# matinmoezzi/MyCobotGym

Hardware: AMD Instinct MI355X
Metric: env-steps/sec (whole node), MyCobot Reach, N_envs=8192/GPU (higher is better)
Workload: dtype f64

## Files before the change

### mycobotgym_amd/csrc/mcg_dynamics.hpp

```cpp
#pragma once
#ifndef MCG_DUP
#define MCG_DUP 0
#endif

#include <type_traits>
#include <hip/hip_runtime.h>
#include "mcg.h"

namespace mcg {

typedef double real;

constexpr int NB = 12;
constexpr int AXK[NB] = {2, 0, 0, 0, 2, 0, 1, 1, 1, 1, 1, 1};
constexpr int AXS[NB] = {-1, -1, 1, -1, -1, -1, 1, -1, -1, 1, 1, 1};
constexpr int PAR[NB] = {-1, 0, 1, 2, 3, 4, 5, 6, 5, 8, 5, 5};
constexpr real MINVAL = 1e-15, MINIMP = 1e-4, MAXIMP = 0.9999;

#define MCG_DEV __device__ __forceinline__

enum { ST_LOAD = 0, ST_CTRL, ST_TRIG, ST_RNE, ST_ACT, ST_CRB, ST_ROWS, ST_G0, ST_NEWTON, ST_EULER, ST_COLLIDE, ST_CUBE,
       ST_COUPLED, ST_CUBE_FIN, ST_POST, ST_N_BUILD, ST_N_FACTOR, ST_N_SOLVE, ST_N_CHECK, ST_E_RHS, ST_R_AX5, ST_R_CONNECT, ST_R_LIMITS, ST_C_MASK, ST_C_ASSEMBLE, ST_C_SCHUR, ST_C_SOLVE, ST_C_CHECK, ST_C_LS, ST_W2_WAIT1, ST_W2_COLLIDE, ST_W2_CUBE, ST_W2_WAIT2, ST_W1_WAIT, ST_A_ENTRY, ST_A_G, ST_A_TWIST, ST_A_LOOP, ST_A_MAP, ST_A_STORE,
       ST_CO_SETUP, ST_CO_ROWS, ST_CO_H0, ST_CO_RESID, ST_CO_ASM, ST_CO_FACTOR, ST_CO_SOLVE, ST_CO_CHECK, ST_CO_LS, ST_CO_OUT, ST_CO_IDLE,
       ST_X_S1C, ST_X_NUMBERS, ST_X_S2, ST_S_S1B, ST_S_MESH, ST_S_S1C, ST_S_NUMBERS,
// ... 117 lines not shown
  pc = fma(z, pc, T.t[11]); pc = fma(z, pc, T.t[12]);
  pc = fma(z, pc, T.t[13]); pc = fma(z, pc, T.t[14]);
  const real cr = fma(z * z, pc, fma(z, -0.5, 1.0));
  const int q = (int)k;
  const real s0 = (q & 1) ? cr : sr, c0 = (q & 1) ? sr : cr;
  s = (q & 2) ? -s0 : s0;
  c = ((q + 1) & 2) ? -c0 : c0;
}

MCG_DEV real impedance(const real* par, real dist) {
  const real d0 = par[2], dmax = par[3], width = par[4], mid = par[5], power = par[6];
  real imp;
  if (d0 == dmax || width <= MINVAL) imp = 0.5 * (d0 + dmax);
  else {
    const real x = fabs(dist) * par[7];
    real y;
    if (power == 2) {
      const real u = 1 - x;
      y = (x <= mid) ? par[8] * (x * x) : 1 - par[9] * (u * u);
    } else y = x;
    imp = d0 + y * (dmax - d0);
    imp = (x >= 1) ? dmax : imp;
    imp = (x == 0) ? d0 : imp;
  }
  return fmin(fmax(imp, MINIMP), MAXIMP);
}

constexpr int tri(int i, int j) { return i >= j ? i * (i + 1) / 2 + j : j * (j + 1) / 2 + i; }

struct Pattern { bool nz[NB][NB]; };

constexpr bool is_ancestor_or_self(int a, int i) {
  while (i >= 0) { if (i == a) return true; i = PAR[i]; }
  return false;
}
constexpr Pattern symbolic(bool with_constraints, bool fill = true) {
  Pattern P{};
  for (int i = 0; i < NB; i++) for (int j = 0; j <= i; j++) P.nz[i][j] = is_ancestor_or_self(j, i);
  if (with_constraints) {
    constexpr int grp[2][3] = {{6, 7, 10}, {8, 9, 11}};
    for (int g = 0; g < 2; g++) for (int a = 0; a < 3; a++) for (int b = 0; b < 3; b++) {
      int i = grp[g][a], j = grp[g][b];
      if (i >= j) P.nz[i][j] = true;
    }
    for (int g = 0; g < 2; g++) for (int a = 0; a < 3; a++) for (int j = 0; j < 6; j++) P.nz[grp[g][a]][j] = true;
    P.nz[8][6] = true;
// ... 355 lines not shown
          for (int k = 0; k < 3; k++) cmc[p][k] += h3[k] + m * r[k];
          for (int k = 0; k < 6; k++) cI[p][k] += add[k];
        }
        pin(cm[p]); pin3(cmc[p]); pin6(cI[p]);
      }
      asm volatile("" ::: "memory");
      MCG_FENCE();
    });
}

template <class LS>
MCG_DEV void euler_accel(ModelPtr Pm, real h, const LS MS, const real* a, real* rhs) {
  real Mh[NB * (NB + 1) / 2], dinv[NB];
  static_for<NB>([&](auto I) { constexpr int i = I;
    static_for<i + 1>([&](auto Jj) { constexpr int j = Jj; if constexpr (PAT_M.nz[i][j]) Mh[tri(i, j)] = MS.ld(LDS_M + tri(i, j)); }); });
  static_for<NB>([&](auto I) { constexpr int i = I; real sacc = 0;
    static_for<NB>([&](auto Jj) { constexpr int j = Jj;
      if constexpr (PAT_M.nz[i > j ? i : j][i > j ? j : i]) sacc = fma(Mh[tri(i, j)], a[j], sacc); }); rhs[i] = sacc; });
  { ModelPtr Q = launder(Pm); static_for<NB>([&](auto I) { constexpr int i = I; Mh[tri(i, i)] = fma(h, Q->body[i].damping, Mh[tri(i, i)]); }); }
  ldl_factor<PAT_M>(Mh, dinv);
  ldl_solve<PAT_M>(Mh, dinv, rhs);
}

struct NoSplit { static constexpr bool enabled = false, rne_remote = false, factor_remote = false, early_heq = false, warm_lds = false, mesh_split = false, solve_remote = false,
                                       trig_once = false;
                 static constexpr int QB = 0, QDB = 0, FS = 0, WARM = 0, QLAG = 0; };
struct SplitMain { static constexpr bool enabled = true, rne_remote = true, factor_remote = true, early_heq = true, warm_lds = true, mesh_split = false, solve_remote = true,
                                         trig_once = true;
                   static constexpr int QB = LDS_QB, QDB = LDS_QDB, FS = LDS_FS, WARM = LDS_WARM, QLAG = LDS_QLAG; };
struct SplitMainLocal : SplitMain { static constexpr bool solve_remote = false; };
struct SplitMainOwnTrig : SplitMain { static constexpr bool trig_once = false; };

template <int FIRST, class LS, class QF>
MCG_DEV void trig_exchange(const LS MS, QF q_of, real* sn, real* cs) {
  {
    const TrigC T = load_trig();
    static_for<4>([&](auto I) { constexpr int i = FIRST + I; real s, c; sincos_cw(T, AXS[i] * q_of(std::integral_constant<int, i>{}), s, c); MS.st(LDS_SN + i, s); MS.st(LDS_CS + i, c); });
  }
  __syncthreads();
  static_for<NB>([&](auto I) { constexpr int i = I; sn[i] = MS.ld(LDS_SN + i); cs[i] = MS.ld(LDS_CS + i); });
}

template <class SPL, class LS>
MCG_DEV void build_H(const LS MS, real* H, const bool* act_, const real* Dl) {
  static_for<NB>([&](auto I) { constexpr int i = I;
    static_for<i + 1>([&](auto Jj) { constexpr int j = Jj;
      if constexpr (PAT_E.nz[i][j]) {
        H[tri(i, j)] = MS.ld(LDS_HEQ + tri(i, j));
        if constexpr (SPL::early_heq && PAT_M.nz[i][j]) H[tri(i, j)] += MS.ld(LDS_M + tri(i, j));
      } else if constexpr (PAT_H.nz[i][j]) H[tri(i, j)] = 0.0; }); });
  static_for<10>([&](auto I) { constexpr int j = I; H[tri(j, j)] += act_[j] ? Dl[j] : 0.0; });
}

template <class SPL, class LS>
MCG_DEV bool no_other_rows(ModelPtr Pm, const LS MS) {
  real jr[10][2];
  { ModelPtr Q = launder(Pm); static_for<10>([&](auto I) { constexpr int j = I; if constexpr (j != 6 && j != 8) { jr[j][0] = Q->jnt_range[j][0]; jr[j][1] = Q->jnt_range[j][1]; } }); }
  bool other = false;
  static_for<10>([&](auto I) { constexpr int j = I;
// ... 22 lines not shown
  f0 = s0 * nu0; f1 = s1 * nu1;
}

MCG_DEV void gear_rows_solve(real* x, const real* z6, const real* z8, real Dl6, real arefl6, real sgl6, real Dl8, real arefl8, real sgl8) {
  const bool v6 = sgl6 != 0, v8 = sgl8 != 0, both = v6 && v8;
  const real D0 = v6 ? Dl6 : (v8 ? Dl8 : 1.0), D1 = both ? Dl8 : 1.0;
  const real ar0 = v6 ? arefl6 : arefl8, ar1 = both ? arefl8 : 0.0;
  const real s0 = v6 ? sgl6 : sgl8, s1 = both ? sgl8 : 0.0;
  const real xa0 = v6 ? x[6] : (v8 ? x[8] : 0.0), xa1 = both ? x[8] : 0.0;
  real W00 = v6 ? z6[6] : (v8 ? z8[8] : 0.0), W01 = both ? z6[8] : 0.0;
  const real W11 = both ? z8[8] : 0.0;
  W01 *= s0 * s1;
  const real rb0 = s0 * xa0 - ar0, rb1 = s1 * xa1 - ar1;
  real f0, f1;
  limit_pair(v6 || v8, both, D0, D1, s0, s1, rb0, rb1, W00, W01, W11, f0, f1);
  const real g6 = v6 ? f0 : 0.0, g8 = v6 ? f1 : f0;
  static_for<NB>([&](auto I) { constexpr int i = I; x[i] = fma(-z8[i], g8, fma(-z6[i], g6, x[i])); });
}

MCG_DEV bool bad_value(real x) { return !(fabs(x) <= 1e10); }

template <class LS, class CPL = NoCoupling, class WLD = NoWeld, class SPL = NoSplit, bool COMMIT = true>
MCG_DEV bool robot_substep(ModelPtr Pm, Robot& S, real* qlag6, const LS MS, CPL* CP = nullptr, const WLD* WD = nullptr,
                           Robot* next = nullptr) {
  MCG_COUNT(CN_SUBSTEP);
  if constexpr (SPL::enabled) __syncthreads();
  const real h = launder(Pm)->timestep;
  real cs[NB], sn[NB];
  if constexpr (SPL::trig_once) trig_exchange<0>(MS, [&](auto I) { return S.q[I]; }, sn, cs);
  else {
    const TrigC T = load_trig();
    static_for<NB>([&](auto I) { constexpr int i = I; sincos_cw(T, AXS[i] * S.q[i], sn[i], cs[i]); });
  }
  if constexpr (!(SPL::warm_lds && !CPL::enabled)) static_for<6>([&](auto I) { constexpr int i = I; qlag6[i] = S.q[i]; });
  static_for<NB>([&](auto I) { constexpr int i = I; pin(sn[i]); pin(cs[i]); });
  MCG_FENCE();

  MCG_TICK(ST_TRIG);
  real fs[NB];
  if constexpr (SPL::rne_remote) { static_for<NB>([&](auto I) { constexpr int i = I; fs[i] = 0; }); }
  else rne_bias(Pm, cs, sn, S.qd, fs);
  MCG_TICK(ST_RNE);
  {
    ModelPtr Q = launder(Pm);
    static_for<6>([&](auto I) {
      constexpr int u = I;
      real c = fmin(fmax(S.ctrl[u], Q->act_ctrlrange[u][0]), Q->act_ctrlrange[u][1]);
      real f = Q->act_gain[u] * c + Q->act_bias[u][0] + Q->act_bias[u][1] * S.q[u] + Q->act_bias[u][2] * S.qd[u];
      fs[u] += fmin(fmax(f, Q->act_forcerange[u][0]), Q->act_forcerange[u][1]);
    });
    const real c0 = Q->tendon_coef[0], c1 = Q->tendon_coef[1];
    real len = c0 * S.q[6] + c1 * S.q[8], vel = c0 * S.qd[6] + c1 * S.qd[8];
    real c = fmin(fmax(S.ctrl[6], Q->act_ctrlrange[6][0]), Q->act_ctrlrange[6][1]);
    real f = Q->act_gain[6] * c + Q->act_bias[6][0] + Q->act_bias[6][1] * len + Q->act_bias[6][2] * vel;
    f = fmin(fmax(f, Q->act_forcerange[6][0]), Q->act_forcerange[6][1]);
    fs[6] += c0 * f; fs[8] += c1 * f;
  }
  static_for<NB>([&](auto I) { constexpr int i = I; pin(fs[i]); });
  if constexpr (SPL::solve_remote) static_for<8>([&](auto K) { constexpr int k = K; MS.st(LDS_RACT + k, fs[RACT_DOF[k]]); });
  MCG_FENCE();

  MCG_TICK(ST_ACT);
  if constexpr (!SPL::enabled) crb_to_lds(Pm, cs, sn, MS);
  MCG_TICK(ST_CRB);
  real ax5[6][3];
  static_for<6>([&](auto I) {
    constexpr int i = I;
    for (int k = 0; k < 3; k++) ax5[i][k] = 0;
    ax5[i][AXK[i]] = AXS[i];
    static_for<5 - i>([&](auto Jj) {
      constexpr int j = i + 1 + Jj;
      real t[3]; rot_down<AXK[j]>(cs[j], sn[j], ax5[i], t);
      for (int k = 0; k < 3; k++) ax5[i][k] = t[k];
    });
  });
  MCG_TICK_PIN(ax5[0], 3); MCG_TICK_PIN(ax5[1], 3); MCG_TICK_PIN(ax5[2], 3); MCG_TICK_PIN(ax5[3], 3); MCG_TICK_PIN(ax5[4], 3);
  MCG_TICK(ST_R_AX5);
  real Jc[2][3][9];
  real Dc[2], arefc[2][3];
  static_for<2>([&](auto Sd) {
    constexpr int sd = Sd; constexpr int g = 6 + 2 * sd, fi = 7 + 2 * sd, hg = 10 + sd;
    ModelPtr Q = launder(Pm);
    real rg[3], rh[3], rf[3], an1[3], an2[3], par[10];
    ldc<3>(Q->body[g].r, rg); ldc<3>(Q->body[hg].r, rh); ldc<3>(Q->body[fi].r, rf);
    ldc<3>(Q->eq_anchor1[sd], an1); ldc<3>(Q->eq_anchor2[sd], an2); ldc<10>(Q->eq_par[sd], par);
    real t[3], t2[3], o_f[3], p1[3], p2[3];
    rot_up<1>(cs[g], sn[g], rf, t);
    for (int k = 0; k < 3; k++) o_f[k] = rg[k] + t[k];
    rot_up<1>(cs[fi], sn[fi], an1, t2); rot_up<1>(cs[g], sn[g], t2, t);
    for (int k = 0; k < 3; k++) p1[k] = o_f[k] + t[k];
    rot_up<1>(cs[hg], sn[hg], an2, t);
    for (int k = 0; k < 3; k++) p2[k] = rh[k] + t[k];
    const real pos[3] = {p1[0] - p2[0], p1[1] - p2[1], p1[2] - p2[2]};
    static_for<6>([&](auto I) { constexpr int i = I; real c3[3]; cross(ax5[i], pos, c3); for (int k = 0; k < 3; k++) Jc[sd][k][i] = c3[k]; });
    Jc[sd][0][6] = AXS[g] * (p1[2] - rg[2]);   Jc[sd][2][6] = -AXS[g] * (p1[0] - rg[0]);
    Jc[sd][0][7] = AXS[fi] * (p1[2] - o_f[2]); Jc[sd][2][7] = -AXS[fi] * (p1[0] - o_f[0]);
    Jc[sd][0][8] = -AXS[hg] * (p2[2] - rh[2]); Jc[sd][2][8] = AXS[hg] * (p2[0] - rh[0]);
    Jc[sd][1][6] = Jc[sd][1][7] = Jc[sd][1][8] = 0;
    const real imp = impedance(par, sqrt(dot3(pos, pos)));
    Dc[sd] = imp * rcp_nr(fmax(MINVAL * imp, (1 - imp) * Q->eq_diag[sd]));
    static_for<3>([&](auto Kk) {
      constexpr int k = Kk;
      real vel = 0;
      static_for<6>([&](auto I) { constexpr int i = I; vel = fma(Jc[sd][k][i], S.qd[i], vel); });
      if constexpr (k != 1) vel += Jc[sd][k][6] * S.qd[g] + Jc[sd][k][7] * S.qd[fi] + Jc[sd][k][8] * S.qd[hg];
      arefc[sd][k] = -par[1] * vel - par[0] * imp * pos[k];
    });
    pin(Dc[sd]); pin3(arefc[sd]);
    for (int k = 0; k < 3; k++) { pin3(&Jc[sd][k][0]); pin3(&Jc[sd][k][3]); pin3(&Jc[sd][k][6]); }
    MCG_FENCE();
  });
  real Dj, arefj;
  {
    ModelPtr Q = launder(Pm);
    real par[10]; ldc<10>(Q->eq_par[2], par);
    const real pos = S.q[6] - S.q[8];
    const real imp = impedance(par, pos);
    Dj = imp * rcp_nr(fmax(MINVAL * imp, (1 - imp) * Q->eq_diag[2]));
    arefj = -par[1] * (S.qd[6] - S.qd[8]) - par[0] * imp * pos;
  }
  MCG_TICK_PIN(&Dj, 1); MCG_TICK_PIN(&arefj, 1);
  MCG_TICK(ST_R_CONNECT);
  real Dl[10], arefl[10], sgl[10];
  bool any_limit = false;
  real jr[10][2];
  { ModelPtr Q = launder(Pm); static_for<10>([&](auto I) { constexpr int j = I; jr[j][0] = Q->jnt_range[j][0]; jr[j][1] = Q->jnt_range[j][1]; }); }
  static_for<10>([&](auto I) {
    constexpr int j = I;
    const real lo = S.q[j] - jr[j][0], hi = jr[j][1] - S.q[j];
    real dist = (lo < 0) ? lo : 0.0, sg = (lo < 0) ? 1.0 : 0.0;
    dist = (hi < 0) ? hi : dist; sg = (hi < 0) ? -1.0 : sg;
    sgl[j] = sg; Dl[j] = 0; arefl[j] = 0;
    if (__any(sg != 0)) {
      ModelPtr Q = launder(Pm);
      real par[10]; ldc<10>(Q->limit_par[j], par);
      const real imp = impedance(par, dist);
      const real D = imp * rcp_nr(fmax(MINVAL * imp, (1 - imp) * Q->limit_diag[j]));
      const real ar = -par[1] * (sg * S.qd[j]) - par[0] * imp * dist;
      Dl[j] = (sg != 0) ? D : 0.0; arefl[j] = (sg != 0) ? ar : 0.0;
      any_limit = any_limit || (sg != 0);
    }
  });
  static_for<10>([&](auto I) { constexpr int j = I; pin(Dl[j]); pin(arefl[j]); pin(sgl[j]); });
  MCG_FENCE();
  MCG_TICK(ST_R_LIMITS);

  real Jw[6][6], Dw[2] = {0, 0}, arefw[6];
  if constexpr (WLD::enabled) {
    ModelPtr Q = launder(Pm);
    TcpPose X; tcp_forward(Q, S.q, X, true);
    real par[10], rq[4], rp[3]; ldc<10>(Q->weld_par, par); ldc<4>(Q->weld_relquat, rq); ldc<3>(Q->weld_relpos, rp);
    const real ts = Q->weld_torquescale;
    real Rm[9]; quat_to_mat(WD->quat, Rm);
    real cpos[6];
    for (int k = 0; k < 3; k++) cpos[k] = (WD->pos[k] + Rm[3 * k] * rp[0] + Rm[3 * k + 1] * rp[1] + Rm[3 * k + 2] * rp[2]) - X.pos[k];
    real quat[4], quat1[4] = {X.quat[0], -X.quat[1], -X.quat[2], -X.quat[3]}, quat2[4];
    mulquat(WD->quat, rq, quat);
    mulquat(quat1, quat, quat2);
    for (int k = 0; k < 3; k++) cpos[3 + k] = ts * quat2[1 + k];
    static_for<6>([&](auto I) {
      constexpr int j = I;
// ... 264 lines not shown
    static_for<NB>([&](auto I) { constexpr int i = I; dinv[i] = MS.ld(LDS_FDINV + i);
      static_for<i>([&](auto Jj) { constexpr int j = Jj; if constexpr (PAT_M.nz[i][j]) Lf[tri(i, j)] = MS.ld(LDS_FAC + tri(i, j)); }); });
    if constexpr (SPL::solve_remote) {
      if (!remote) { ModelPtr Q = launder(Pm); static_for<NB>([&](auto I) { constexpr int i = I; damp[i] = Q->body[i].damping; }); }
      static_for<NB>([&](auto I) { constexpr int i = I; rhs[i] = damp[i] * a[i]; });
    } else { ModelPtr Q = launder(Pm); static_for<NB>([&](auto I) { constexpr int i = I; rhs[i] = Q->body[i].damping * a[i]; }); }
    ldl_solve<PAT_M>(Lf, dinv, rhs);
    static_for<NB>([&](auto I) { constexpr int i = I; rhs[i] = fma(-h, rhs[i], a[i]); });
  } else {
  MCG_TICK(ST_E_RHS);
  euler_accel(Pm, h, MS, a, rhs);
  }
  real qn[NB], qdn[NB];
  bool bad = false;
  static_for<NB>([&](auto I) { constexpr int i = I;
    real q_old, qd_old;
    if constexpr (SPL::warm_lds && !CPL::enabled) { q_old = MS.ld(SPL::QB + i); qd_old = MS.ld(SPL::QDB + i); if constexpr (i < 6) MS.st(SPL::QLAG + i, q_old); }
    else { q_old = S.q[i]; qd_old = S.qd[i]; }
    qdn[i] = fma(h, rhs[i], qd_old); qn[i] = fma(h, qdn[i], q_old);
    if constexpr (COMMIT) bad = bad || bad_value(qn[i]) || bad_value(qdn[i]) || bad_value(a[i]); });
  if constexpr (COMMIT) {
    if (__any(bad)) {
      static_for<NB>([&](auto I) { constexpr int i = I; qn[i] = sel(bad, 0.0, qn[i]); qdn[i] = sel(bad, 0.0, qdn[i]); a[i] = sel(bad, 0.0, a[i]); });
      static_for<7>([&](auto I) { constexpr int k = I; S.ctrl[k] = sel(bad, 0.0, S.ctrl[k]); });
    }
  }
  static_for<NB>([&](auto I) { constexpr int i = I;
    const real qd_new = qdn[i], q_new = qn[i];
    if constexpr (COMMIT) { S.qd[i] = qd_new; S.q[i] = q_new; if constexpr (SPL::warm_lds && !CPL::enabled) MS.st(SPL::WARM + i, a[i]); else S.warm[i] = a[i]; }
    else { next->qd[i] = qd_new; next->q[i] = q_new; next->warm[i] = a[i]; }
    if constexpr (SPL::enabled && COMMIT) { MS.st(SPL::QB + i, q_new); MS.st(SPL::QDB + i, qd_new); } });
  MCG_TICK_PIN(S.q, NB); MCG_TICK_PIN(S.qd, NB);
  MCG_TICK(ST_EULER);
  if constexpr (SPL::enabled && SPL::mesh_split) { if (ahead) { __syncthreads(); __syncthreads(); } }
  return bad;
}

template <class SPL, int FIRST, class LS>
MCG_DEV void side_trig(const LS MS, real* sn, real* cs) {
  if constexpr (SPL::trig_once) trig_exchange<FIRST>(MS, [&](auto I) { return MS.ld(SPL::QB + I); }, sn, cs);
  else {
    const TrigC T = load_trig();
    static_for<NB>([&](auto I) { constexpr int i = I; sincos_cw(T, AXS[i] * MS.ld(SPL::QB + i), sn[i], cs[i]); });
  }
  static_for<NB>([&](auto I) { constexpr int i = I; pin(sn[i]); pin(cs[i]); });
  MCG_FENCE();
}

template <class SPL = SplitMain, class LS, class SIDE = NoSideWork>
MCG_DEV void helper_substep(ModelPtr Pm, const LS MS, const SIDE& side = SIDE{}) {
  __syncthreads();
  MCG_TICK(ST_H_S1);
  real cs[NB], sn[NB];
  side_trig<SPL, 4>(MS, sn, cs);
  crb_to_lds(Pm, cs, sn, MS);
  static_assert(!SPL::mesh_split, "the four-wave PickAndPlace kernel drives its side waves itself: helper_pre / rne_pre");
  (void)side;
  MCG_TICK(ST_H_CRB);
  __syncthreads();
  MCG_TICK(ST_H_S2);
  if constexpr (SPL::factor_remote) {
    const real h = launder(Pm)->timestep;
    real Mh[NB * (NB + 1) / 2], dinv[NB];
    static_for<NB>([&](auto I) { constexpr int i = I;
      static_for<i + 1>([&](auto Jj) { constexpr int j = Jj; if constexpr (PAT_M.nz[i][j]) Mh[tri(i, j)] = MS.ld(LDS_M + tri(i, j)); }); });
    { ModelPtr Q = launder(Pm); static_for<NB>([&](auto I) { constexpr int i = I; Mh[tri(i, i)] = fma(h, Q->body[i].damping, Mh[tri(i, i)]); }); }
    ldl_factor<PAT_M>(Mh, dinv);
    static_for<NB>([&](auto I) { constexpr int i = I; MS.st(LDS_FDINV + i, dinv[i]);
      static_for<i>([&](auto Jj) { constexpr int j = Jj; if constexpr (PAT_M.nz[i][j]) MS.st(LDS_FAC + tri(i, j), Mh[tri(i, j)]); }); });
    MCG_TICK(ST_H_FACTOR);
    __syncthreads();
    MCG_TICK(ST_H_S3);
  }
}

template <class SPL = SplitMain, class LS, class SIDE = NoSideWork>
MCG_DEV void rne_substep(ModelPtr Pm, const LS MS, const SIDE& side = SIDE{}) {
  __syncthreads();
  MCG_TICK(ST_Q_S1);
  real cs[NB], sn[NB], qd[NB], fs[NB];
  side_trig<SPL, 8>(MS, sn, cs);
  static_for<NB>([&](auto I) { constexpr int i = I; qd[i] = MS.ld(SPL::QDB + i); });
  rne_bias(Pm, cs, sn, qd, fs);
  static_for<NB>([&](auto I) { constexpr int i = I; MS.st(SPL::FS + i, fs[i]); });
  bool remote = false;
  if constexpr (SPL::solve_remote) {
    remote = no_other_rows<SPL>(Pm, MS);
    static_for<NB>([&](auto I) { constexpr int i = I; pin(fs[i]); });
    MCG_FENCE();
  }
  static_assert(!SPL::mesh_split, "the four-wave PickAndPlace kernel drives its side waves itself: helper_pre / rne_pre");
  (void)side;
  MCG_TICK(ST_Q_BIAS);
  __syncthreads();
  MCG_TICK(ST_Q_S2);
  if constexpr (SPL::solve_remote) {
    if (remote) {
      real L[NB * (NB + 1) / 2], dinv[NB], x[NB];
      const bool none[10] = {false, false, false, false, false, false, false, false, false, false};
      const real zero[10] = {0, 0, 0, 0, 0, 0, 0, 0, 0, 0};
      build_H<SPL>(MS, L, none, zero);
      static_for<NB>([&](auto I) { constexpr int i = I; x[i] = 0.0; });
      static_for<8>([&](auto K) { constexpr int k = K; x[RACT_DOF[k]] = MS.ld(LDS_RACT + k); });
      static_for<NB>([&](auto I) { constexpr int i = I; x[i] = MS.ld(LDS_RG0 + i) + (x[i] + fs[i]); });
// ... 175 lines not shown
```

### mycobotgym_amd/csrc/mcg_hip.hip

```cpp
#include <hip/hip_runtime.h>
#include <cstdlib>
#include <cstddef>
#include <cmath>
#include <cstdarg>
#include <cstdio>
#include <cstring>
#include <new>
#include <vector>

#include "mcg.h"
#include "mcg_engine.hpp"
#include "mcg_dynamics.hpp"
#include "mcg_cube.hpp"
#include "mcg_coop.hpp"
#include "model_gen.h"
#include "polytopes_gen.h"

using namespace mcg;

namespace {

struct Env {
  Robot R;
  real qlag6[6], goal[3], epret;
// ... 93 lines not shown
MCG_DEV void mocap_target(const Cfg& C, ModelPtr P, const real* qlag6, const float* act, Weld& W) {
  TcpPose X; tcp_forward(P, qlag6, X, false);
  for (int k = 0; k < 3; k++) W.pos[k] = X.pos[k] + (real)(act[k] * 0.1f);
  const real fq[4] = {0.5, -0.5, -0.5, 0.5};
  for (int k = 0; k < 4; k++) {
    const real qt = C.fetch ? fq[k] : (real)act[3 + k];
    const real dq = qt - X.quat[k];
    W.quat[k] = X.quat[k] + dq;
  }
  normalize4(W.quat);
}

#ifndef MCG_SOLVE_REMOTE_CTRLS
#define MCG_SOLVE_REMOTE_CTRLS (1 << MCG_CTRL_JOINT)
#endif

template <int CONTROLLER, bool SPLIT>
__global__ __launch_bounds__(SPLIT ? 192 : 64) void step_reach_kernel(Cfg C, View V, const mcg_model* __restrict__ Pg,
                                                                      const float* __restrict__ actions, mcg_step_out O) {
  typedef std::conditional_t<SPLIT, std::conditional_t<(MCG_SOLVE_REMOTE_CTRLS >> CONTROLLER) & 1, SplitMain, SplitMainLocal>, NoSplit> Split;
  __shared__ real lds[SPLIT ? LDS_SLOTS_SPLIT : LDS_SLOTS][64];
  const int lane = threadIdx.x & 63;
  const LaneScratch MS(&lds[0][lane]);
  const ModelPtr P = as_model_ptr(Pg);
  const int i = blockIdx.x * 64 + lane;
  if (i >= C.n) return;
  if constexpr (SPLIT) {
    if (threadIdx.x >= 64) {
      MCG_TICK_INIT();
      if constexpr (CONTROLLER == MCG_CTRL_IK) {
        if (threadIdx.x < 128) {
          for (int c = 0; c < C.control_steps; c++) { __syncthreads(); __syncthreads(); for (int s = 0; s < C.frame_skip; s++) helper_substep<Split>(P, MS); }
        } else {
          float act[8];
          _Pragma("unroll") for (int k = 0; k < 8; k++) {
            const float x = (k < C.act_dim) ? actions[(size_t)i * C.act_dim + (k < C.act_dim ? k : 0)] : 0.f;
            act[k] = fminf(fmaxf(x, -1.f), 1.f);
          }
          real tpos[3], tquat[4];
          for (int c = 0; c < C.control_steps; c++) {
            __syncthreads();
            real ql[6]; EefPose X;
            for (int k = 0; k < 6; k++) ql[k] = MS.ld(LDS_QLAG + k);
            eef_forward(P, ql, X, true);
            if (c == 0) {
              for (int k = 0; k < 3; k++) tpos[k] = X.pos[k] + (real)(act[k] * 0.2f);
              if (C.fetch) { tquat[0] = 0; tquat[1] = -0.707; tquat[2] = 0; tquat[3] = 0.707; }
// ... 53 lines not shown
      real e[3], qr[4], cur[4];
      for (int k = 0; k < 3; k++) e[k] = (real)(act[3 + k] * 0.5f);
      euler2quat(e, qr); mat2quat(X.mat, cur); mulquat(qr, cur, tquat);
    }
    const real grip = C.grip_center + (real)act_last * C.grip_range;
    for (int c = 0; c < C.control_steps; c++) {
      if (c > 0) eef_forward(P, E.qlag6, X, true);
      real dq[6];
      ik_delta(X, tpos, tquat, dq);
      for (int k = 0; k < 6; k++) E.R.ctrl[k] += dq[k];
      E.R.ctrl[6] = grip;
      if (c == 0) for (int k = 0; k < 7; k++) E.R.ctrl[k] = sel(bad0, 0.0, E.R.ctrl[k]);
      MCG_TICK(ST_CTRL);
      for (int s = 0; s < C.frame_skip; s++) hadbad |= robot_substep<LaneScratch, NoCoupling, NoWeld, Split>(P, E.R, E.qlag6, MS);
    }
  } else if constexpr (CONTROLLER == MCG_CTRL_MOCAP) {
    Weld W; mocap_target(C, P, E.qlag6, act, W);
    E.R.ctrl[6] = sel(bad0, 0.0, C.grip_center + (real)act_last * C.grip_range);
    MCG_TICK(ST_CTRL);
    for (int s = 0; s < C.frame_skip; s++) hadbad |= robot_substep<LaneScratch, NoCoupling, Weld, Split>(P, E.R, E.qlag6, MS, nullptr, &W);
  } else {
    for (int k = 0; k < 7; k++) E.R.ctrl[k] = sel(bad0, 0.0, (real)act[k]);
    MCG_TICK(ST_CTRL);
    for (int s = 0; s < C.frame_skip; s++) hadbad |= robot_substep<LaneScratch, NoCoupling, NoWeld, Split>(P, E.R, E.qlag6, MS);
  }

  if constexpr (SPLIT) static_for<NB>([&](auto I) { constexpr int k = I; E.R.warm[k] = MS.ld(LDS_WARM + k); if constexpr (k < 6) E.qlag6[k] = MS.ld(LDS_QLAG + k); });
  hadbad |= guard_robot(E.R, E.qlag6);
  if (__any(hadbad)) {
    bool zero = true;
    for (int k = 0; k < NB; k++) zero = zero && E.R.q[k] == 0.0 && E.R.qd[k] == 0.0;
    for (int k = 0; k < 6; k++) E.qlag6[k] = sel(hadbad && zero, 0.0, E.qlag6[k]);
  }
  count_event(C, 1, hadbad);
  int i_tail = i; asm volatile("" : "+v"(i_tail));
  load_episode(V, i_tail, E);
  if (C.block_gripper) {
    E.R.q[7] = 0; E.R.q[9] = 0;
    for (int k = 0; k < 6; k++) E.qlag6[k] = E.R.q[k];
  }
  real obs[10], ag[3];
  observe_reach(C, P, E, obs, ag);
  real dx = ag[0] - E.goal[0], dy = ag[1] - E.goal[1], dz = ag[2] - E.goal[2];
  const real dist = sqrt(dx * dx + dy * dy + dz * dz);
  const bool succ = dist < C.distance_threshold;
  const real rew = sel(C.reward_type == MCG_REWARD_SPARSE, -(real)(float)(dist > C.distance_threshold), -dist);
  E.elapsed++; E.eplen++; E.epret += rew;
// ... 129 lines not shown
  real Rl[9], eul[3];
  quat_to_mat(E.qlag7 + 3, Rl); mat2euler(Rl, eul);
  for (int k = 0; k < 3; k++) {
    obs[k] = X.pos[k]; obs[3 + k] = E.qlag7[k]; obs[6 + k] = E.qlag7[k] - X.pos[k];
    obs[11 + k] = eul[k];
    obs[14 + k] = E.Cb.vel[k] * C.dt - gv[k];
    obs[17 + k] = (Rl[3*k]*E.Cb.vel[3] + Rl[3*k+1]*E.Cb.vel[4] + Rl[3*k+2]*E.Cb.vel[5]) * C.dt;
    obs[20 + k] = gv[k];
    ag[k] = E.qlag7[k];
  }
  obs[9] = E.R.q[6]; obs[10] = E.R.q[8];
  obs[23] = E.R.qd[6] * C.dt; obs[24] = E.R.qd[8] * C.dt;
}

MCG_DEV void hide_object(real* obs, real* ag) {
  const real o[10] = {obs[0], obs[1], obs[2], obs[9], obs[10], obs[20], obs[21], obs[22], obs[23], obs[24]};
  for (int k = 0; k < 10; k++) obs[k] = o[k];
  for (int k = 0; k < 3; k++) ag[k] = o[k];
}

constexpr int XCH_FS = PNP_SLOTS;
constexpr int PNP_SLOTS_DUAL = PNP_SLOTS_LDS;
static_assert(PNP_SLOTS_DUAL * PNP_LANES * 8 <= 160 * 1024, "LDS of a CU");
struct SplitPnp { static constexpr bool enabled = true, rne_remote = true, factor_remote = false, early_heq = true, warm_lds = false, mesh_split = true, solve_remote = false, trig_once = false;
                  static constexpr int QB = XCH_Q, QDB = XCH_QD, FS = XCH_FS, WARM = 0, QLAG = 0, MASK0 = MP_MASK; };

MCG_DEV bool flag_coupled(real f) { return (((int)f) & 2) != 0; }
MCG_DEV bool flag_cube_bad(real f) { return (((int)f) & 8) != 0; }

struct PubHook {
  static constexpr bool enabled = false, publishes = true;
  const PnpScratch S;
  MCG_DEV void publish(const real* g0, const real* Dl, const real* arefl, const real* sgl, const real* qd, const real* warm, bool flags_known) const {
    const bool flag = !flags_known || flag_coupled(S.ld(XCH_FLAG));
    if (__any(flag)) {
      if (flag) {
        static_for<NB>([&](auto I) { constexpr int k = I; S.st(PUB_G0 + k, g0[k]); S.st(PUB_WARM + k, warm[k]); });
        static_for<10>([&](auto I) { constexpr int j = I; S.st(PUB_SD + j, sgl[j] * Dl[j]); S.st(pub_aref(j), arefl[j]); });
      }
    }
  }
};

MCG_DEV void cube_to_lds(const PnpScratch MS, const Cube& Cb) {
  for (int k = 0; k < 3; k++) MS.st(XCH_CB + k, Cb.pos[k]);
  for (int k = 0; k < 4; k++) MS.st(XCH_CB + 3 + k, Cb.quat[k]);
  for (int k = 0; k < 6; k++) { MS.st(XCH_CB + 7 + k, Cb.vel[k]); MS.st(XCH_CB + 13 + k, Cb.warm[k]); }
// ... 557 lines not shown
  memcpy(C.init_qpos, c->init_qpos, sizeof(C.init_qpos));
  memcpy(C.init_qvel, c->init_qvel, sizeof(C.init_qvel));
  memcpy(C.init_ctrl, c->init_ctrl, sizeof(C.init_ctrl));
  C.seed = c->seed; C.env_id_offset = c->env_id_offset;
  C.dr_enable = c->dr_enable && c->has_object;
  C.block_gripper = c->block_gripper;
  for (int k = 0; k < 3; k++) C.qpos0_cube[k] = m->body[12].r[k];
  C.qpos0_cube[3] = 1; C.qpos0_cube[4] = C.qpos0_cube[5] = C.qpos0_cube[6] = 0;
  C.dr_mass[0] = c->dr_mass_range[0]; C.dr_mass[1] = c->dr_mass_range[1];
  C.dr_fric[0] = c->dr_friction_range[0]; C.dr_fric[1] = c->dr_friction_range[1];
  e->device = device;
  {
    hipDeviceProp_t prop;
    e->num_cu = (hipGetDeviceProperties(&prop, device) == hipSuccess) ? prop.multiProcessorCount : 256;
    const char* ns = getenv("MCG_NO_SPLIT");
    e->no_split = ns && ns[0] == '1';
    const char* cp = getenv("MCG_COOP_PAIR");
    C.coop_pair = !(cp && cp[0] == '0');
  }
  e->view.n = C.n; e->view.nq = C.nq; e->view.nv = C.nv;
  size_t nd = (size_t)state_doubles(C.nq, C.nv) * C.n;
  hipError_t err = hipMalloc(&e->view.d, nd * sizeof(double));
  if (err == hipSuccess) err = hipMalloc(&e->view.i32, (size_t)3 * C.n * sizeof(int32_t));
  if (err == hipSuccess) err = hipMalloc(&e->d_model, sizeof(mcg_model));
  if (err == hipSuccess) err = hipMalloc(&e->d_cnt, sizeof(mcg_counters));
  if (err == hipSuccess && C.has_object) {
    err = hipMalloc(&e->d_poly, np * sizeof(double));
    if (err == hipSuccess) err = hipMemcpy(e->d_poly, pb, np * sizeof(double), hipMemcpyHostToDevice);
  }
  if (err == hipSuccess) {
    e->render_ok = C.has_object || (polytope_index_ok(pb, np, e->render_why, sizeof(e->render_why)) && polytopes_fit_model(pb, m, e->render_why, sizeof(e->render_why)));
    if (e->render_ok) render_face_table(e, pb);
  }
  if (err == hipSuccess) err = hipMemset(e->d_cnt, 0, sizeof(mcg_counters));
  if (err == hipSuccess) C.cnt = e->d_cnt;
  if (err == hipSuccess) err = hipMemset(e->view.d, 0, nd * sizeof(double));
  if (err == hipSuccess) err = hipMemset(e->view.i32, 0, (size_t)3 * C.n * sizeof(int32_t));
  if (err == hipSuccess) {
    std::vector<double> ones((size_t)2 * C.n, 1.0);
    err = hipMemcpy(e->view.row(e->view.rows().dr), ones.data(), ones.size() * sizeof(double), hipMemcpyHostToDevice);
  }
  if (err == hipSuccess) {
    mcg_model mm = *m;
    if (!(mm.contact_rpy > 0.0)) mm.contact_rpy = 2.0;
    if (C.hidden) mm.cube_half[0] = mm.cube_half[1] = mm.cube_half[2] = 0.0;
    err = hipMemcpy(e->d_model, &mm, sizeof(mcg_model), hipMemcpyHostToDevice);
  }
  if (err != hipSuccess) { mcg_destroy(e); return mcg_fail(MCG_ERR_HIP, "mcg_create: %s", hipGetErrorString(err)); }
  *out = e;
  return MCG_OK;
}

void mcg_destroy(mcg_env* e) {
  if (!e) return;
  (void)hipSetDevice(e->device);
  if (e->view.d) (void)hipFree(e->view.d);
  if (e->view.i32) (void)hipFree(e->view.i32);
  if (e->d_model) (void)hipFree(e->d_model);
  if (e->d_poly) (void)hipFree(e->d_poly);
  if (e->d_cnt) (void)hipFree(e->d_cnt);
  if (e->d_faces) (void)hipFree(e->d_faces);
  delete e;
}

#ifdef MCG_STAGE_CLOCKS
extern "C" int mcg_debug_wg_stat(unsigned long long* out, int n, int clear) {
  if (hipDeviceSynchronize() != hipSuccess) return MCG_ERR_HIP;
  if (out && hipMemcpyFromSymbol(out, HIP_SYMBOL(mcg::g_wg_stat), sizeof(unsigned long long) * n) != hipSuccess) return MCG_ERR_HIP;
  if (clear) { static unsigned long long z[4096 * 4]; if (hipMemcpyToSymbol(HIP_SYMBOL(mcg::g_wg_stat), z, sizeof(z)) != hipSuccess) return MCG_ERR_HIP; }
// ... 125 lines not shown
```

Baseline: 43.22 million.

## Precompute impedance row records on host and prefetch scalar model constants

Adds a host-derived ModelRows block appended to the device model that holds per-constraint impedance records (span, constant-impedance value, mode), actuator bias and tendon coefficients. The split main wave loads these records through the scalar constant path and pins them in SGPRs, and it loads trig constants and the timestep before the barrier. The aim is to shorten the scalar-load and ALU latency in the connect, coupling and limit row setup and to overlap those loads with the sync. An optional actuator-hoist path, off by default, would also precompute control terms once per frame. The risks are extra SGPR pressure and the added complexity of the model layout.

```diff
diff --git a/mycobotgym_amd/csrc/mcg_dynamics.hpp b/mycobotgym_amd/csrc/mcg_dynamics.hpp
--- a/mycobotgym_amd/csrc/mcg_dynamics.hpp
+++ b/mycobotgym_amd/csrc/mcg_dynamics.hpp
@@ -163,6 +163,66 @@
     imp = d0 + y * (dmax - d0);
     imp = (x >= 1) ? dmax : imp;
     imp = (x == 0) ? d0 : imp;
+  }
+  return fmin(fmax(imp, MINIMP), MAXIMP);
+}
+
+struct ImpRec { real K, B, d0, dmax, span , rwidth, mid, a, b, diag, cimp , mode ; };
+constexpr real IMP_CONST = 0, IMP_POW1 = 1, IMP_POW2 = 2;
+struct ModelRows { ImpRec connect[2], coupling, limit[10]; real act[7][4], tendon[2]; };
+struct ModelDev { mcg_model m; ModelRows rows; };
+static_assert(sizeof(mcg_model) % 8 == 0 && offsetof(ModelDev, rows) == sizeof(mcg_model), "the records follow the model directly");
+inline ImpRec derive_row(const double* par, double diag) {
+  ImpRec r;
+  r.K = par[0]; r.B = par[1]; r.d0 = par[2]; r.dmax = par[3]; r.span = par[3] - par[2]; r.rwidth = par[7]; r.mid = par[5];
+  r.a = par[8]; r.b = par[9]; r.diag = diag; r.cimp = 0.5 * (par[2] + par[3]);
+  r.mode = (par[2] == par[3] || par[4] <= MINVAL) ? IMP_CONST : (par[6] == 2 ? IMP_POW2 : IMP_POW1);
+  return r;
+}
+inline void derive_rows(const mcg_model& m, ModelRows& x) {
+  for (int k = 0; k < 2; k++) x.connect[k] = derive_row(m.eq_par[k], m.eq_diag[k]);
+  x.coupling = derive_row(m.eq_par[2], m.eq_diag[2]);
+  for (int j = 0; j < 10; j++) x.limit[j] = derive_row(m.limit_par[j], m.limit_diag[j]);
+  for (int u = 0; u < 7; u++) { x.act[u][0] = m.act_bias[u][1]; x.act[u][1] = m.act_bias[u][2]; x.act[u][2] = m.act_forcerange[u][0]; x.act[u][3] = m.act_forcerange[u][1]; }
+  x.tendon[0] = m.tendon_coef[0]; x.tendon[1] = m.tendon_coef[1];
+}
+typedef const __attribute__((address_space(4))) ModelRows* RowsPtr;
+MCG_DEV RowsPtr rows_of(ModelPtr P) { RowsPtr r = (RowsPtr)(P + 1); asm volatile("" : "+s"(r)); return r; }
+typedef const __attribute__((address_space(4))) ImpRec* RecPtr;
+MCG_DEV ImpRec load_rec(RecPtr p) {
+  ImpRec r;
+  r.K = p->K; r.B = p->B; r.d0 = p->d0; r.dmax = p->dmax; r.span = p->span; r.rwidth = p->rwidth; r.mid = p->mid; r.a = p->a; r.b = p->b;
+  r.diag = p->diag; r.cimp = p->cimp; r.mode = p->mode;
+  return r;
+}
+MCG_DEV void pin_s(real& a, real& b, real& c, real& d) { asm volatile("" : "+s"(a), "+s"(b), "+s"(c), "+s"(d)); }
+MCG_DEV void pin_rec(ImpRec& r) { pin_s(r.K, r.B, r.d0, r.dmax); pin_s(r.span, r.rwidth, r.mid, r.a); pin_s(r.b, r.diag, r.cimp, r.mode); }
+MCG_DEV void act_const(ModelPtr Pm, const real* ctrl, real* g) {
+  ModelPtr Q = launder(Pm);
+  static_for<7>([&](auto I) { constexpr int u = I;
+    const real c = fmin(fmax(ctrl[u], Q->act_ctrlrange[u][0]), Q->act_ctrlrange[u][1]);
+    g[u] = fma(Q->act_gain[u], c, Q->act_bias[u][0]); });
+}
+struct Act4 { real a[4][4]; };
+struct Act3 { real a[3][4], tendon[2]; };
+MCG_DEV Act4 load_act4(RowsPtr X) { Act4 r; for (int u = 0; u < 4; u++) for (int k = 0; k < 4; k++) r.a[u][k] = X->act[u][k]; return r; }
+MCG_DEV Act3 load_act3(RowsPtr X) { Act3 r; for (int u = 0; u < 3; u++) for (int k = 0; k < 4; k++) r.a[u][k] = X->act[4 + u][k]; r.tendon[0] = X->tendon[0]; r.tendon[1] = X->tendon[1]; return r; }
+struct S1Pre { TrigC T; real h; };
+MCG_DEV S1Pre load_s1(ModelPtr Pm) { S1Pre r; r.T = load_trig(); r.h = launder(Pm)->timestep; return r; }
+MCG_DEV real impedance_rec(const ImpRec& r, real dist) {
+  real imp;
+  if (r.mode == IMP_CONST) imp = r.cimp;
+  else {
+    const real x = fabs(dist) * r.rwidth;
+    real y = x;
+    if (r.mode == IMP_POW2) {
+      const real u = 1 - x;
+      const real ylo = r.a * (x * x), yhi = 1 - r.b * (u * u);
+      y = (x <= r.mid) ? ylo : yhi;
+    }
+    imp = r.d0 + y * r.span;
+    imp = (x >= 1) ? r.dmax : imp;
+    imp = (x == 0) ? r.d0 : imp;
   }
   return fmin(fmax(imp, MINIMP), MAXIMP);
 }
@@ -564,19 +624,31 @@
   ldl_solve<PAT_M>(Mh, dinv, rhs);
 }
 
+#ifndef MCG_R8_ROWS
+#define MCG_R8_ROWS true
+#endif
+#ifndef MCG_R8_ACT
+#define MCG_R8_ACT false
+#endif
+#ifndef MCG_R8_S1
+#define MCG_R8_S1 true
+#endif
+#ifndef MCG_R8_OPAQUE
+#define MCG_R8_OPAQUE true
+#endif
 struct NoSplit { static constexpr bool enabled = false, rne_remote = false, factor_remote = false, early_heq = false, warm_lds = false, mesh_split = false, solve_remote = false,
-                                       trig_once = false;
+                                       trig_once = false, row_records = false, act_hoist = false, s1_ahead = false;
                  static constexpr int QB = 0, QDB = 0, FS = 0, WARM = 0, QLAG = 0; };
 struct SplitMain { static constexpr bool enabled = true, rne_remote = true, factor_remote = true, early_heq = true, warm_lds = true, mesh_split = false, solve_remote = true,
-                                         trig_once = true;
+                                         trig_once = true, row_records = MCG_R8_ROWS, act_hoist = MCG_R8_ACT, s1_ahead = MCG_R8_S1;
                    static constexpr int QB = LDS_QB, QDB = LDS_QDB, FS = LDS_FS, WARM = LDS_WARM, QLAG = LDS_QLAG; };
-struct SplitMainLocal : SplitMain { static constexpr bool solve_remote = false; };
+struct SplitMainLocal : SplitMain { static constexpr bool solve_remote = false, row_records = false, act_hoist = false, s1_ahead = false; };
 struct SplitMainOwnTrig : SplitMain { static constexpr bool trig_once = false; };
 
 template <int FIRST, class LS, class QF>
-MCG_DEV void trig_exchange(const LS MS, QF q_of, real* sn, real* cs) {
+MCG_DEV void trig_exchange(const LS MS, QF q_of, real* sn, real* cs, const TrigC* Tpre = nullptr) {
   {
-    const TrigC T = load_trig();
+    const TrigC T = Tpre ? *Tpre : load_trig();
     static_for<4>([&](auto I) { constexpr int i = FIRST + I; real s, c; sincos_cw(T, AXS[i] * q_of(std::integral_constant<int, i>{}), s, c); MS.st(LDS_SN + i, s); MS.st(LDS_CS + i, c); });
   }
   __syncthreads();
@@ -645,12 +717,17 @@
 
 template <class LS, class CPL = NoCoupling, class WLD = NoWeld, class SPL = NoSplit, bool COMMIT = true>
 MCG_DEV bool robot_substep(ModelPtr Pm, Robot& S, real* qlag6, const LS MS, CPL* CP = nullptr, const WLD* WD = nullptr,
-                           Robot* next = nullptr) {
+                           Robot* next = nullptr, real* actg = nullptr) {
   MCG_COUNT(CN_SUBSTEP);
+  S1Pre pre;
+  if constexpr (SPL::s1_ahead) pre = load_s1(Pm);
   if constexpr (SPL::enabled) __syncthreads();
-  const real h = launder(Pm)->timestep;
+  real h;
+  if constexpr (SPL::s1_ahead) h = pre.h; else h = launder(Pm)->timestep;
   real cs[NB], sn[NB];
-  if constexpr (SPL::trig_once) trig_exchange<0>(MS, [&](auto I) { return S.q[I]; }, sn, cs);
+  Act4 actA;
+  if constexpr (SPL::act_hoist) { actA = load_act4(rows_of(Pm)); MCG_FENCE(); }
+  if constexpr (SPL::trig_once) trig_exchange<0>(MS, [&](auto I) { return S.q[I]; }, sn, cs, SPL::s1_ahead ? &pre.T : nullptr);
   else {
     const TrigC T = load_trig();
     static_for<NB>([&](auto I) { constexpr int i = I; sincos_cw(T, AXS[i] * S.q[i], sn[i], cs[i]); });
@@ -664,7 +741,22 @@
   if constexpr (SPL::rne_remote) { static_for<NB>([&](auto I) { constexpr int i = I; fs[i] = 0; }); }
   else rne_bias(Pm, cs, sn, S.qd, fs);
   MCG_TICK(ST_RNE);
-  {
+  if constexpr (SPL::act_hoist) {
+    const Act3 actB = load_act3(rows_of(Pm)); MCG_FENCE();
+    static_for<4>([&](auto I) { constexpr int u = I;
+      const real f = fma(actA.a[u][1], S.qd[u], fma(actA.a[u][0], S.q[u], actg[u]));
+      fs[u] += fmin(fmax(f, actA.a[u][2]), actA.a[u][3]); });
+    static_for<4>([&](auto I) { constexpr int i = I; pin(fs[i]); });
+    MCG_FENCE();
+    static_for<2>([&](auto I) { constexpr int u = 4 + I;
+      const real f = fma(actB.a[u - 4][1], S.qd[u], fma(actB.a[u - 4][0], S.q[u], actg[u]));
+      fs[u] += fmin(fmax(f, actB.a[u - 4][2]), actB.a[u - 4][3]); });
+    const real c0 = actB.tendon[0], c1 = actB.tendon[1];
+    real len = c0 * S.q[6] + c1 * S.q[8], vel = c0 * S.qd[6] + c1 * S.qd[8];
+    real f = fma(actB.a[2][1], vel, fma(actB.a[2][0], len, actg[6]));
+    f = fmin(fmax(f, actB.a[2][2]), actB.a[2][3]);
+    fs[6] += c0 * f; fs[8] += c1 * f;
+  } else {
     ModelPtr Q = launder(Pm);
     static_for<6>([&](auto I) {
       constexpr int u = I;
@@ -706,7 +798,12 @@
     ModelPtr Q = launder(Pm);
     real rg[3], rh[3], rf[3], an1[3], an2[3], par[10];
     ldc<3>(Q->body[g].r, rg); ldc<3>(Q->body[hg].r, rh); ldc<3>(Q->body[fi].r, rf);
-    ldc<3>(Q->eq_anchor1[sd], an1); ldc<3>(Q->eq_anchor2[sd], an2); ldc<10>(Q->eq_par[sd], par);
+    ldc<3>(Q->eq_anchor1[sd], an1); ldc<3>(Q->eq_anchor2[sd], an2);
+    ImpRec rec;
+    if constexpr (SPL::row_records) {
+      pin_s(rg[0], rg[1], rg[2], rh[0]); pin_s(rh[1], rh[2], rf[0], rf[1]); pin_s(rf[2], an1[0], an1[1], an1[2]); asm volatile("" : "+s"(an2[0]), "+s"(an2[1]), "+s"(an2[2]));
+      rec = load_rec(&rows_of(Pm)->connect[sd]); MCG_FENCE();
+    } else ldc<10>(Q->eq_par[sd], par);
     real t[3], t2[3], o_f[3], p1[3], p2[3];
     rot_up<1>(cs[g], sn[g], rf, t);
     for (int k = 0; k < 3; k++) o_f[k] = rg[k] + t[k];
@@ -720,14 +817,16 @@
     Jc[sd][0][7] = AXS[fi] * (p1[2] - o_f[2]); Jc[sd][2][7] = -AXS[fi] * (p1[0] - o_f[0]);
     Jc[sd][0][8] = -AXS[hg] * (p2[2] - rh[2]); Jc[sd][2][8] = AXS[hg] * (p2[0] - rh[0]);
     Jc[sd][1][6] = Jc[sd][1][7] = Jc[sd][1][8] = 0;
-    const real imp = impedance(par, sqrt(dot3(pos, pos)));
-    Dc[sd] = imp * rcp_nr(fmax(MINVAL * imp, (1 - imp) * Q->eq_diag[sd]));
+    real imp, eqd, parB, parK;
+    if constexpr (SPL::row_records) { pin_rec(rec); MCG_FENCE(); imp = impedance_rec(rec, sqrt(dot3(pos, pos))); eqd = rec.diag; parB = rec.B; parK = rec.K; }
+    else { imp = impedance(par, sqrt(dot3(pos, pos))); eqd = Q->eq_diag[sd]; parB = par[1]; parK = par[0]; }
+    Dc[sd] = imp * rcp_nr(fmax(MINVAL * imp, (1 - imp) * eqd));
     static_for<3>([&](auto Kk) {
       constexpr int k = Kk;
       real vel = 0;
       static_for<6>([&](auto I) { constexpr int i = I; vel = fma(Jc[sd][k][i], S.qd[i], vel); });
       if constexpr (k != 1) vel += Jc[sd][k][6] * S.qd[g] + Jc[sd][k][7] * S.qd[fi] + Jc[sd][k][8] * S.qd[hg];
-      arefc[sd][k] = -par[1] * vel - par[0] * imp * pos[k];
+      arefc[sd][k] = -parB * vel - parK * imp * pos[k];
     });
     pin(Dc[sd]); pin3(arefc[sd]);
     for (int k = 0; k < 3; k++) { pin3(&Jc[sd][k][0]); pin3(&Jc[sd][k][3]); pin3(&Jc[sd][k][6]); }
@@ -735,12 +834,19 @@
   });
   real Dj, arefj;
   {
+    const real pos = S.q[6] - S.q[8];
+    if constexpr (SPL::row_records) {
+      ImpRec rec = load_rec(&rows_of(Pm)->coupling); pin_rec(rec); MCG_FENCE();
+      const real imp = impedance_rec(rec, pos);
+      Dj = imp * rcp_nr(fmax(MINVAL * imp, (1 - imp) * rec.diag));
+      arefj = -rec.B * (S.qd[6] - S.qd[8]) - rec.K * imp * pos;
+    } else {
     ModelPtr Q = launder(Pm);
     real par[10]; ldc<10>(Q->eq_par[2], par);
-    const real pos = S.q[6] - S.q[8];
     const real imp = impedance(par, pos);
     Dj = imp * rcp_nr(fmax(MINVAL * imp, (1 - imp) * Q->eq_diag[2]));
     arefj = -par[1] * (S.qd[6] - S.qd[8]) - par[0] * imp * pos;
+    }
   }
   MCG_TICK_PIN(&Dj, 1); MCG_TICK_PIN(&arefj, 1);
   MCG_TICK(ST_R_CONNECT);
@@ -748,18 +854,35 @@
   bool any_limit = false;
   real jr[10][2];
   { ModelPtr Q = launder(Pm); static_for<10>([&](auto I) { constexpr int j = I; jr[j][0] = Q->jnt_range[j][0]; jr[j][1] = Q->jnt_range[j][1]; }); }
+  ImpRec rec6, rec8;
+  if constexpr (SPL::row_records) {
+    static_for<5>([&](auto I) { constexpr int j = 2 * I; pin_s(jr[j][0], jr[j][1], jr[j + 1][0], jr[j + 1][1]); });
+    rec6 = load_rec(&rows_of(Pm)->limit[6]); MCG_FENCE();
+  }
   static_for<10>([&](auto I) {
     constexpr int j = I;
+    if constexpr (SPL::row_records && j == 6) { pin_rec(rec6); rec8 = load_rec(&rows_of(Pm)->limit[8]); MCG_FENCE(); }
+    if constexpr (SPL::row_records && j == 8) { pin_rec(rec8); MCG_FENCE(); }
     const real lo = S.q[j] - jr[j][0], hi = jr[j][1] - S.q[j];
     real dist = (lo < 0) ? lo : 0.0, sg = (lo < 0) ? 1.0 : 0.0;
     dist = (hi < 0) ? hi : dist; sg = (hi < 0) ? -1.0 : sg;
     sgl[j] = sg; Dl[j] = 0; arefl[j] = 0;
     if (__any(sg != 0)) {
+      real D, ar;
+      if constexpr (SPL::row_records) {
+        ImpRec rec;
+        if constexpr (j == 6) rec = rec6; else if constexpr (j == 8) rec = rec8;
+        else { rec = load_rec(&rows_of(Pm)->limit[j]); pin_rec(rec); MCG_FENCE(); }
+        const real imp = impedance_rec(rec, dist);
+        D = imp * rcp_nr(fmax(MINVAL * imp, (1 - imp) * rec.diag));
+        ar = -rec.B * (sg * S.qd[j]) - rec.K * imp * dist;
+      } else {
       ModelPtr Q = launder(Pm);
       real par[10]; ldc<10>(Q->limit_par[j], par);
       const real imp = impedance(par, dist);
-      const real D = imp * rcp_nr(fmax(MINVAL * imp, (1 - imp) * Q->limit_diag[j]));
-      const real ar = -par[1] * (sg * S.qd[j]) - par[0] * imp * dist;
+      D = imp * rcp_nr(fmax(MINVAL * imp, (1 - imp) * Q->limit_diag[j]));
+      ar = -par[1] * (sg * S.qd[j]) - par[0] * imp * dist;
+      }
       Dl[j] = (sg != 0) ? D : 0.0; arefl[j] = (sg != 0) ? ar : 0.0;
       any_limit = any_limit || (sg != 0);
     }
@@ -1070,6 +1193,11 @@
   if constexpr (COMMIT) {
     if (__any(bad)) {
       static_for<NB>([&](auto I) { constexpr int i = I; qn[i] = sel(bad, 0.0, qn[i]); qdn[i] = sel(bad, 0.0, qdn[i]); a[i] = sel(bad, 0.0, a[i]); });
+      if constexpr (SPL::act_hoist) {
+        const real zero[7] = {0, 0, 0, 0, 0, 0, 0}; real g0[7];
+        act_const(Pm, zero, g0);
+        static_for<7>([&](auto I) { constexpr int k = I; actg[k] = sel(bad, g0[k], actg[k]); });
+      } else
       static_for<7>([&](auto I) { constexpr int k = I; S.ctrl[k] = sel(bad, 0.0, S.ctrl[k]); });
     }
   }
@@ -1085,8 +1213,8 @@
 }
 
 template <class SPL, int FIRST, class LS>
-MCG_DEV void side_trig(const LS MS, real* sn, real* cs) {
-  if constexpr (SPL::trig_once) trig_exchange<FIRST>(MS, [&](auto I) { return MS.ld(SPL::QB + I); }, sn, cs);
+MCG_DEV void side_trig(const LS MS, real* sn, real* cs, const TrigC* Tpre = nullptr) {
+  if constexpr (SPL::trig_once) trig_exchange<FIRST>(MS, [&](auto I) { return MS.ld(SPL::QB + I); }, sn, cs, Tpre);
   else {
     const TrigC T = load_trig();
     static_for<NB>([&](auto I) { constexpr int i = I; sincos_cw(T, AXS[i] * MS.ld(SPL::QB + i), sn[i], cs[i]); });
@@ -1097,10 +1225,12 @@
 
 template <class SPL = SplitMain, class LS, class SIDE = NoSideWork>
 MCG_DEV void helper_substep(ModelPtr Pm, const LS MS, const SIDE& side = SIDE{}) {
+  TrigC Tpre;
+  if constexpr (SPL::s1_ahead) Tpre = load_trig();
   __syncthreads();
   MCG_TICK(ST_H_S1);
   real cs[NB], sn[NB];
-  side_trig<SPL, 4>(MS, sn, cs);
+  side_trig<SPL, 4>(MS, sn, cs, SPL::s1_ahead ? &Tpre : nullptr);
   crb_to_lds(Pm, cs, sn, MS);
   static_assert(!SPL::mesh_split, "the four-wave PickAndPlace kernel drives its side waves itself: helper_pre / rne_pre");
   (void)side;
@@ -1124,10 +1254,12 @@
 
 template <class SPL = SplitMain, class LS, class SIDE = NoSideWork>
 MCG_DEV void rne_substep(ModelPtr Pm, const LS MS, const SIDE& side = SIDE{}) {
+  TrigC Tpre;
+  if constexpr (SPL::s1_ahead) Tpre = load_trig();
   __syncthreads();
   MCG_TICK(ST_Q_S1);
   real cs[NB], sn[NB], qd[NB], fs[NB];
-  side_trig<SPL, 8>(MS, sn, cs);
+  side_trig<SPL, 8>(MS, sn, cs, SPL::s1_ahead ? &Tpre : nullptr);
   static_for<NB>([&](auto I) { constexpr int i = I; qd[i] = MS.ld(SPL::QDB + i); });
   rne_bias(Pm, cs, sn, qd, fs);
   static_for<NB>([&](auto I) { constexpr int i = I; MS.st(SPL::FS + i, fs[i]); });
diff --git a/mycobotgym_amd/csrc/mcg_hip.hip b/mycobotgym_amd/csrc/mcg_hip.hip
--- a/mycobotgym_amd/csrc/mcg_hip.hip
+++ b/mycobotgym_amd/csrc/mcg_hip.hip
@@ -139,7 +139,7 @@
   __shared__ real lds[SPLIT ? LDS_SLOTS_SPLIT : LDS_SLOTS][64];
   const int lane = threadIdx.x & 63;
   const LaneScratch MS(&lds[0][lane]);
-  const ModelPtr P = as_model_ptr(Pg);
+  const ModelPtr P = (Split::row_records && MCG_R8_OPAQUE) ? launder(as_model_ptr(Pg)) : as_model_ptr(Pg);
   const int i = blockIdx.x * 64 + lane;
   if (i >= C.n) return;
   if constexpr (SPLIT) {
@@ -239,7 +239,16 @@
   } else {
     for (int k = 0; k < 7; k++) E.R.ctrl[k] = sel(bad0, 0.0, (real)act[k]);
     MCG_TICK(ST_CTRL);
-    for (int s = 0; s < C.frame_skip; s++) hadbad |= robot_substep<LaneScratch, NoCoupling, NoWeld, Split>(P, E.R, E.qlag6, MS);
+    real actg[7];
+    if constexpr (Split::act_hoist) act_const(P, E.R.ctrl, actg);
+    for (int s = 0; s < C.frame_skip; s++) hadbad |= robot_substep<LaneScratch, NoCoupling, NoWeld, Split>(P, E.R, E.qlag6, MS, nullptr, nullptr, nullptr, actg);
+    if constexpr (Split::act_hoist) {
+      int i_act = i; asm volatile("" : "+v"(i_act));
+      _Pragma("unroll") for (int k = 0; k < 7; k++) {
+        const float x = (k < C.act_dim) ? actions[(size_t)i_act * C.act_dim + (k < C.act_dim ? k : 0)] : 0.f;
+        E.R.ctrl[k] = sel(hadbad, 0.0, (real)fminf(fmaxf(x, -1.f), 1.f));
+      }
+    }
   }
 
   if constexpr (SPLIT) static_for<NB>([&](auto I) { constexpr int k = I; E.R.warm[k] = MS.ld(LDS_WARM + k); if constexpr (k < 6) E.qlag6[k] = MS.ld(LDS_QLAG + k); });
@@ -415,7 +424,7 @@
 constexpr int XCH_FS = PNP_SLOTS;
 constexpr int PNP_SLOTS_DUAL = PNP_SLOTS_LDS;
 static_assert(PNP_SLOTS_DUAL * PNP_LANES * 8 <= 160 * 1024, "LDS of a CU");
-struct SplitPnp { static constexpr bool enabled = true, rne_remote = true, factor_remote = false, early_heq = true, warm_lds = false, mesh_split = true, solve_remote = false, trig_once = false;
+struct SplitPnp { static constexpr bool enabled = true, rne_remote = true, factor_remote = false, early_heq = true, warm_lds = false, mesh_split = true, solve_remote = false, trig_once = false, row_records = false, act_hoist = false, s1_ahead = false;
                   static constexpr int QB = XCH_Q, QDB = XCH_QD, FS = XCH_FS, WARM = 0, QLAG = 0, MASK0 = MP_MASK; };
 
 MCG_DEV bool flag_coupled(real f) { return (((int)f) & 2) != 0; }
@@ -1019,7 +1028,7 @@
   size_t nd = (size_t)state_doubles(C.nq, C.nv) * C.n;
   hipError_t err = hipMalloc(&e->view.d, nd * sizeof(double));
   if (err == hipSuccess) err = hipMalloc(&e->view.i32, (size_t)3 * C.n * sizeof(int32_t));
-  if (err == hipSuccess) err = hipMalloc(&e->d_model, sizeof(mcg_model));
+  if (err == hipSuccess) err = hipMalloc(&e->d_model, sizeof(ModelDev));
   if (err == hipSuccess) err = hipMalloc(&e->d_cnt, sizeof(mcg_counters));
   if (err == hipSuccess && C.has_object) {
     err = hipMalloc(&e->d_poly, np * sizeof(double));
@@ -1041,7 +1050,8 @@
     mcg_model mm = *m;
     if (!(mm.contact_rpy > 0.0)) mm.contact_rpy = 2.0;
     if (C.hidden) mm.cube_half[0] = mm.cube_half[1] = mm.cube_half[2] = 0.0;
-    err = hipMemcpy(e->d_model, &mm, sizeof(mcg_model), hipMemcpyHostToDevice);
+    ModelDev md; md.m = mm; derive_rows(md.m, md.rows);
+    err = hipMemcpy(e->d_model, &md, sizeof(ModelDev), hipMemcpyHostToDevice);
   }
   if (err != hipSuccess) { mcg_destroy(e); return mcg_fail(MCG_ERR_HIP, "mcg_create: %s", hipGetErrorString(err)); }
   *out = e;
```

After: 43.61 million, median of 6. No clear change (+0.9%).
